# protocol/vdf

Hardware: AMD Instinct MI355X
Metric: MSM GPoints/s at 2^20 (Pallas, Pedersen-commitment MSM of Nova prove_step); prove_step/s in `prove_step` (higher is better)
Workload: dtype u32

## Files before the change

### bindings/rust/vdf-hip-sys/src/lib.rs

```rust
#![allow(non_camel_case_types, non_snake_case)]
use std::os::raw::{c_char, c_int, c_uint, c_void};

#[repr(C)] pub struct VdfCtx { _private: [u8; 0] }
#[repr(C)] pub struct VdfBases { _private: [u8; 0] }
#[repr(C)] pub struct VdfShape { _private: [u8; 0] }
#[repr(C)] pub struct VdfMsmJob { _private: [u8; 0] }
#[repr(C)] pub struct VdfPp { _private: [u8; 0] }
#[repr(C)] pub struct VdfCircuits { _private: [u8; 0] }
#[repr(C)] pub struct VdfProof { _private: [u8; 0] }
#[repr(C)] pub struct VdfSnark { _private: [u8; 0] }
#[repr(C)] pub struct VdfCs { _private: [u8; 0] }
#[repr(C)] pub struct VdfCustomChain { _private: [u8; 0] }

#[repr(C)] #[derive(Clone, Copy, Debug, PartialEq, Eq)] pub struct VdfFe { pub l: [u64; 4] }
#[repr(C)] #[derive(Clone, Copy, Debug, PartialEq, Eq)] pub struct VdfAffine { pub x: VdfFe, pub y: VdfFe }
#[repr(C)] #[derive(Clone, Copy, Debug, PartialEq, Eq)] pub struct VdfJac { pub x: VdfFe, pub y: VdfFe, pub z: VdfFe }
#[repr(C)] #[derive(Clone, Copy, Debug, PartialEq, Eq)] pub struct VdfState { pub x: VdfFe, pub y: VdfFe, pub i: VdfFe }
pub type VdfAllgatherFn = Option<unsafe extern "C" fn(user: *mut c_void, send: *const c_void, recv: *mut c_void, bytes: usize, stream: *mut c_void) -> c_int>;
#[repr(C)] #[derive(Clone, Copy)] pub struct VdfStepCircuit { pub arity: usize, pub synthesize: Option<unsafe extern "C" fn(self_: *mut c_void, cs: *mut VdfCs, z_in: *const u32, z_out: *mut u32) -> c_int>, pub self_: *mut c_void }
#[repr(C)] #[derive(Clone, Copy, Debug)] pub struct VdfNovaStepInfo { pub comm_W1: VdfAffine, pub X1: [VdfFe; 2], pub comm_T1: VdfAffine, pub comm_T2: VdfAffine, pub r1: [u64; 4], pub r2: [u64; 4] }
#[repr(C)] #[derive(Clone, Copy, Debug)] pub struct VdfNovaAugInputs { pub params: VdfFe, pub i: VdfFe, pub z0: [VdfFe; 3], pub zi: [VdfFe; 3], pub U_comm_W: VdfAffine, pub U_comm_E: VdfAffine, pub U_u: VdfFe, pub U_X: [VdfFe; 2], pub u_comm_W: VdfAffine, pub u_X: [VdfFe; 2], pub T: VdfAffine }
#[repr(C)] #[derive(Clone, Copy, Debug)] pub struct VdfKernelEvent { pub name: [c_char; 24], pub bytes: f64, pub start_ms: f64, pub end_ms: f64 }
#[repr(C)] #[derive(Clone, Copy, Debug)] pub struct VdfHipTuning { pub struct_size: u32, pub msm_direct: i32, pub direct_priority: i32, pub direct_fused: i32, pub light_priority: i32, pub accumulate_fill: i32, pub accumulate_lds: i32, pub slice_len: i32, pub part_bits: i32, pub reduction: i32, pub reduction_quads: i32, pub heavy_min: i32, pub giant_span: i32, pub nifs_lanes: i32, pub shim_cache: i32, pub nifs_fused: i32, pub fold_u128: i32, pub fixup_serial: i32, pub sort_staged: i32, pub glv: i32 }
#[repr(C)] #[derive(Clone, Copy, Debug)] pub struct VdfNovaTuning { pub struct_size: u32, pub flags: u32, pub digit_budget_bytes: u64, pub digit_window: i32, pub early_rows: i32, pub stencil: i32, pub small_window: i32, pub big_window: i32, pub packed_commit: i32, pub lookahead_early: i32, pub gate_accumulate: i32, pub fold_on_rows: i32, pub nifs_ahead: i32, pub early_row_parts: i32, pub lookahead_priority: i32, pub side_accumulate_fill: i32, pub verbose: i32, pub compress_queues: i32, pub rows_at_challenge: i32, pub fold_fused: i32, pub periodic_rows: i32, pub custom_ahead: i32 }
#[repr(C)] #[derive(Clone, Copy, Debug, PartialEq, Eq)] pub struct VdfNovaRoParams { pub struct_size: u32, pub family: i32, pub width: i32, pub full_rounds: i32, pub partial_rounds: i32, pub alpha: i32, pub challenge_bits: i32, pub hash_bits: i32 }
#[repr(C)] #[derive(Clone, Copy, Debug)] pub struct VdfIpaOpening { pub weight: VdfFe, pub k: c_int, pub log_m: c_int, pub lo: *const VdfFe, pub hi: *const VdfFe, pub pattern: *const VdfFe }
#[repr(C)] #[derive(Clone, Copy, Debug)] pub struct VdfNovaStreamStats { pub eval_ms: f64, pub after_eval_ms: f64, pub max_backlog: u64, pub steps: u64 }
#[repr(C)] #[derive(Clone, Copy, Debug, PartialEq, Eq)] pub struct VdfTapeOp { pub op: u8, pub dst: u8, pub a: u8, pub b: u8 }
#[repr(C)] #[derive(Clone, Copy, Debug)] pub struct VdfRoundTape { pub ops: *const VdfTapeOp, pub n_ops: usize, pub consts: *const VdfFe, pub n_consts: usize, pub n_slots: u32, pub n_vars: u32, pub n_cons: u32, pub n_inv: u32, pub n_adv: u32 }
#[repr(C)] #[derive(Clone, Copy)] pub struct VdfRoundBody { pub n_inv: usize, pub n_carry: usize, pub n_adv: usize, pub body: Option<unsafe extern "C" fn(self_: *mut c_void, cs: *mut VdfCs, j: u32, inv: *const u32, carry: *const u32, cur: *const u32, next: *const u32, carry_out: *mut u32) -> c_int>, pub self_: *mut c_void }
#[repr(C)] #[derive(Clone, Copy)] pub struct VdfWalkBody { pub n_inv: usize, pub n_adv: usize, pub body: Option<unsafe extern "C" fn(self_: *mut c_void, cs: *mut VdfCs, j: u32, inv: *const u32, next: *const u32, cur_out: *mut u32) -> c_int>, pub self_: *mut c_void }
#[repr(C)] #[derive(Clone, Copy, Debug, PartialEq, Eq)] pub struct VdfPeriodicTerm { pub kind: u8, pub c0: u8, pub c1: u8, pub pad: u8, pub col: u32 }
#[repr(C)] #[derive(Clone, Copy, Debug)] pub struct VdfPeriodicRows { pub n_cons: u32, pub n_vars: u32, pub j0: u64, pub row_start: *const u16, pub terms: *const VdfPeriodicTerm, pub n_terms: usize, pub consts: *const VdfFe, pub n_consts: usize }
#[repr(C)] #[derive(Clone, Copy, Debug, PartialEq, Eq)] pub struct VdfPowStep { pub src: u8, pub squarings: u8, pub mul: u8, pub dst: u8 }

#[link(name = "vdf_hip")]
extern "C" {
    pub fn vdf_ctx_create(device_ids: *const c_int, n_devices: c_int, out: *mut *mut VdfCtx) -> c_int;
// ... 287 lines not shown
```

### include/vdf_hip.h

```cpp
#ifndef VDF_HIP_H
#define VDF_HIP_H

#include <stdbool.h>
#include <stddef.h>
#include <stdint.h>

#ifdef __cplusplus
extern "C" {
#endif

typedef struct { uint64_t l[4]; } vdf_fe;
typedef struct { vdf_fe x, y; } vdf_affine;
typedef struct { vdf_fe x, y, z; } vdf_jac;
typedef struct { vdf_fe x, y, i; } vdf_state;

typedef struct vdf_ctx vdf_ctx;
typedef struct vdf_bases vdf_bases;
typedef struct vdf_shape vdf_shape;

enum {
  VDF_OK = 0,
  VDF_ERR_BAD_ARG = 1,
  VDF_ERR_BAD_LENGTH = 2,
  VDF_ERR_NONCANONICAL = 3,
// ... 246 lines not shown
  int32_t accumulate_fill;
  int32_t accumulate_lds;
  int32_t slice_len;
  int32_t part_bits;
  int32_t reduction;
  int32_t reduction_quads;
  int32_t heavy_min;
  int32_t giant_span;
  int32_t nifs_lanes;
  int32_t shim_cache;
  int32_t nifs_fused;
  int32_t fold_u128;
  int32_t fixup_serial;
  int32_t sort_staged;
  int32_t glv;
} vdf_hip_tuning;
int  vdf_hip_tuning_get(vdf_hip_tuning* out);
int  vdf_hip_tuning_set(const vdf_hip_tuning* in);
int  vdf_ctx_set_accumulate_fill(vdf_ctx* ctx, int workgroups_per_cu);
int  vdf_ctx_clock_probe(vdf_ctx* ctx, int iters, double* shader_mhz, double* kernel_ms);
int  vdf_dev_alloc(vdf_ctx* ctx, size_t bytes, void** out);
int  vdf_dev_free(vdf_ctx* ctx, void* p);
int  vdf_dev_mem_info(vdf_ctx* ctx, size_t* free_bytes, size_t* total_bytes);
int  vdf_dev_memcpy(vdf_ctx* ctx, void* dst, const void* src, size_t bytes);
int  vdf_ptr_download(void* dst, const void* src, size_t bytes);
int  vdf_host_alloc(vdf_ctx* ctx, size_t bytes, void** out);
int  vdf_host_free(vdf_ctx* ctx, void* p);
int  vdf_dev_memset(vdf_ctx* ctx, void* dst, int value, size_t bytes);
const char* vdf_version(void);

// ... 5 lines not shown
```

### vdf_amd/csrc/abi.hip

```cpp
#include <algorithm>
#include <cstring>
#include <cstdio>
#include <cstdlib>
#include <thread>
#include <functional>
#include <map>
#include <array>
#include <new>
#include <memory>
#include <atomic>
#include <deque>
#include <mutex>
#include <initializer_list>
#include <utility>
#include "internal.h"
#include "fe.cuh"

using vdf::Status;

namespace {

thread_local std::string g_create_err;
std::mutex g_default_mu;
vdf_ctx* g_default_ctx = nullptr;
// ... 76 lines not shown
  if (ctx) ctx->err = s.msg; else g_create_err = s.msg;
  return s.code;
}


std::once_flag g_tune_once;
std::mutex g_tune_mu;
std::deque<vdf_hip_tuning> g_tune_snapshots;
std::atomic<const vdf_hip_tuning*> g_tune{nullptr};
vdf_hip_tuning tuning_defaults() {
  vdf_hip_tuning t{};
  t.struct_size = (uint32_t)sizeof(vdf_hip_tuning);
  t.msm_direct = 1; t.direct_priority = 2; t.direct_fused = 1; t.light_priority = 3; t.accumulate_fill = 0;
  t.accumulate_lds = 0; t.slice_len = 0; t.part_bits = -1; t.reduction = 1; t.reduction_quads = 0; t.heavy_min = 0;
  t.giant_span = 0; t.nifs_lanes = 0; t.shim_cache = 0; t.nifs_fused = 1; t.fold_u128 = 1;
  t.fixup_serial = 1; t.sort_staged = 1; t.glv = 1;
  return t;
}
bool tuning_valid(const vdf_hip_tuning& t) {
  auto in = [](int v, int lo, int hi) { return v >= lo && v <= hi; };
  return in(t.msm_direct, 0, 1) && in(t.direct_priority, 0, 3) && in(t.direct_fused, 0, 1) && in(t.light_priority, 0, 3) &&
         in(t.accumulate_fill, 0, 3) && in(t.accumulate_lds, 0, 65536) && in(t.slice_len, 0, 65536) && in(t.part_bits, -1, 19) &&
         in(t.reduction, 0, 1) && (t.reduction_quads == 0 || in(t.reduction_quads, 64, 65536)) &&
         (t.heavy_min == 0 || in(t.heavy_min, 1, 4096)) && (t.giant_span == 0 || in(t.giant_span, 16, 1 << 20)) &&
         (t.nifs_lanes == 0 || t.nifs_lanes == 1 || t.nifs_lanes == 4 || t.nifs_lanes == 8) && in(t.shim_cache, 0, 64) &&
         in(t.nifs_fused, 0, 1) && in(t.fold_u128, 0, 1) && in(t.fixup_serial, 0, 1) && in(t.sort_staged, 0, 1) && in(t.glv, 0, 1);
}
void tuning_publish(const vdf_hip_tuning& t) {
  g_tune_snapshots.push_back(t);
  g_tune_snapshots.back().struct_size = (uint32_t)sizeof(vdf_hip_tuning);
  g_tune.store(&g_tune_snapshots.back(), std::memory_order_release);
}
void tuning_from_env() {
  vdf_hip_tuning t = tuning_defaults();
  const struct { const char* name; int32_t* field; } vars[] = {
      {"VDF_MSM_DIRECT", &t.msm_direct}, {"VDF_MSM_DIRECT_PRIO", &t.direct_priority}, {"VDF_MSM_DIRECT_FUSED", &t.direct_fused},
      {"VDF_MSM_LIGHT_PRIO", &t.light_priority}, {"VDF_MSM_ACC_WG", &t.accumulate_fill}, {"VDF_MSM_ACC_LDS", &t.accumulate_lds},
      {"VDF_MSM_L", &t.slice_len}, {"VDF_MSM_PB", &t.part_bits}, {"VDF_MSM_RED", &t.reduction},
      {"VDF_MSM_RED_QUADS", &t.reduction_quads}, {"VDF_MSM_HEAVY_MIN", &t.heavy_min}, {"VDF_MSM_GIANT_SPAN", &t.giant_span},
      {"VDF_NIFS_LANES", &t.nifs_lanes}, {"VDF_SHIM_CACHE", &t.shim_cache}, {"VDF_NIFS_FUSED", &t.nifs_fused}, {"VDF_FOLD_U128", &t.fold_u128},
      {"VDF_MSM_FIXUP_SERIAL", &t.fixup_serial}, {"VDF_MSM_SORT_STAGED", &t.sort_staged}, {"VDF_MSM_GLV", &t.glv}};
  for (const auto& v : vars) {
    const char* e = std::getenv(v.name);
    if (!e || !*e) continue;
    const int32_t old = *v.field;
    *v.field = (int32_t)std::atol(e);
    if (!tuning_valid(t)) *v.field = old;
  }
  std::lock_guard<std::mutex> lock(g_tune_mu);
  tuning_publish(t);
}
}
namespace vdf {
thread_local KSink* tl_ksink = nullptr;
const vdf_hip_tuning& tuning() {
  std::call_once(g_tune_once, tuning_from_env);
// ... 2211 lines not shown
```

### vdf_amd/csrc/msm.hip

```cpp
#include <cstdlib>
#include <cstring>
#include "internal.h"
#include "ec.cuh"
#include "ecq.cuh"

namespace vdf {

static constexpr uint32_t SIGN_BIT = 0x80000000u;

__device__ __forceinline__ void raise_wave_priority(int wave_prio = 3) {
  if (wave_prio >= 3) __builtin_amdgcn_s_setprio(3);
  else if (wave_prio == 2) __builtin_amdgcn_s_setprio(2);
  else if (wave_prio == 1) __builtin_amdgcn_s_setprio(1);
}
static constexpr int ACC_WG_PER_CU = 3;
static constexpr int ACC_WG_FILL = 2;
static constexpr uint32_t HEAVY_MIN = 6;
static constexpr uint32_t GIANT_SPAN = 64;
static constexpr uint32_t GIANT_CHUNK = 32;
static constexpr uint32_t GIANT_PARTS = 256;
static constexpr uint32_t MAX_GIANTS = 192;
__device__ __forceinline__ uint32_t giant_parts(uint32_t span) {
  const uint32_t p = (span + GIANT_CHUNK - 1) / GIANT_CHUNK;
  return p > GIANT_PARTS ? GIANT_PARTS : p;
// ... 228 lines not shown
      const uint32_t mag = d & ~SIGN_BIT;
      if (!mag) continue;
      const uint32_t s = (uint32_t)w % (uint32_t)sets, j = (uint32_t)w / (uint32_t)sets;
      const uint32_t bin = ((set0 + s) << pb) | ((mag - 1) >> fb);
      const uint32_t pos = atomicAdd(&cur[bin], 1u);
      if (SCATTER) { recsP[pos] = (j * tstride + pbase + i) | (d & SIGN_BIT); recsK[pos] = (uint16_t)((mag - 1) & fmask); }
    }
  }
  if (!SCATTER) {
    __syncthreads();
    for (uint32_t b = threadIdx.x; b < bins; b += 256) mine[b] = cur[b];
  }
}

static constexpr uint32_t PART_STAGE_BINS = 512;
template <class SP>
__global__ __launch_bounds__(256) void k_part_staged(PartGroups pg, int is_mont, int c, int windows, int sets, int pb, int fb,
                                                     uint32_t bins, uint32_t chA, uint32_t tstride,
                                                     const uint32_t* __restrict__ countsA, const uint32_t* __restrict__ pstart,
                                                     uint32_t* __restrict__ recsP, uint16_t* __restrict__ recsK, int wave_prio) {
  raise_wave_priority(wave_prio);
  __shared__ uint32_t limbs[9 * 256];
  __shared__ uint32_t cur[PART_STAGE_BINS];
  __shared__ uint32_t tcnt[PART_STAGE_BINS];
  __shared__ uint32_t toff[PART_STAGE_BINS + 1];
  __shared__ uint32_t tpos[PART_STAGE_BINS];
  __shared__ uint32_t stage[256 * 16];
  __shared__ uint32_t skb[256 * 16];
  const uint32_t* mine = countsA + (size_t)blockIdx.x * bins;
  for (uint32_t b = threadIdx.x; b < bins; b += 256) { cur[b] = pstart[b] + mine[b]; tcnt[b] = 0; }
  int g = 0;
// ... 3 lines not shown
  const uint32_t n = pg.n[g];
  const uint32_t lo = (blockIdx.x - blk0) * chA;
  const uint32_t hi = (lo + chA < n) ? lo + chA : n;
  const uint32_t fmask = (1u << fb) - 1u;
  const uint32_t set0 = (uint32_t)g * (uint32_t)sets;
  const uint32_t pbase = pg.off[g];
  const uint32_t per_lane = (bins + 63) / 64;
  Fe<SP> nxt = fe_zero<SP>();
  if (lo + threadIdx.x < hi) nxt = fe_load<SP>(scalars + (size_t)(lo + threadIdx.x) * 8);
  __syncthreads();
  for (uint32_t base = lo; base < hi; base += 256) {
    const uint32_t i = base + threadIdx.x;
    Fe<SP> mags = nxt;
    if (i + 256 < hi) nxt = fe_load<SP>(scalars + (size_t)(i + 256) * 8);
    uint32_t ssign = 0;
    if (i < hi) {
      if (pg.signed_scalars) { ssign = mags.v[7] & SIGN_BIT; mags.v[7] &= ~SIGN_BIT; }
      stage_scalar<SP>(limbs, mags, is_mont);
      DigitIter it{limbs + threadIdx.x, 0u};
      for (int w = 0; w < windows; ++w) {
        const uint32_t mag = it.next(w, c) & ~SIGN_BIT;
        if (!mag) continue;
        atomicAdd(&tcnt[((set0 + (uint32_t)w % (uint32_t)sets) << pb) | ((mag - 1) >> fb)], 1u);
      }
    }
    __syncthreads();
    if (threadIdx.x < 64) {
      uint32_t run = 0;
      const uint32_t b0 = threadIdx.x * per_lane;
      for (uint32_t k = 0; k < per_lane; ++k) if (b0 + k < bins) run += tcnt[b0 + k];
      uint32_t incl = run;
#pragma unroll
      for (int d = 1; d < 64; d <<= 1) { const uint32_t o = __shfl_up(incl, d, 64); if ((int)threadIdx.x >= d) incl += o; }
      uint32_t off = incl - run;
      for (uint32_t k = 0; k < per_lane; ++k) if (b0 + k < bins) { toff[b0 + k] = off; tpos[b0 + k] = off; off += tcnt[b0 + k]; }
      if (threadIdx.x == 63) toff[bins] = incl;
    }
    __syncthreads();
    if (i < hi) {
      DigitIter it{limbs + threadIdx.x, 0u};
      for (int w = 0; w < windows; ++w) {
        const uint32_t d = it.next(w, c) ^ ssign;
        const uint32_t mag = d & ~SIGN_BIT;
        if (!mag) continue;
        const uint32_t s = (uint32_t)w % (uint32_t)sets, j = (uint32_t)w / (uint32_t)sets;
        const uint32_t bin = ((set0 + s) << pb) | ((mag - 1) >> fb);
        const uint32_t p = atomicAdd(&tpos[bin], 1u);
        stage[p] = (j * tstride + pbase + i) | (d & SIGN_BIT);
        skb[p] = ((mag - 1) & fmask) | (bin << 16);
      }
    }
    __syncthreads();
    const uint32_t tile_n = toff[bins];
    for (uint32_t q = threadIdx.x; q < tile_n; q += 256) {
// ... 364 lines not shown
      if (!queued) q.items[atomicAdd(q.count, 1u)] = g;
    }
    return;
  }
  QPoint<P> acc = qpoint_load_lazy<P>(bucket_acc + (size_t)g * 128);
  QPoint<P> nxt = qpoint_load_lazy<P>(heads + (size_t)(tf + 1) * 128);
  for (uint32_t t = tf + 1; t <= tl; ++t) {
    const QPoint<P> cur = nxt;
    if (t < tl) nxt = qpoint_load_lazy<P>(heads + (size_t)(t + 1) * 128);
    acc = qpoint_add<P>(acc, cur);
  }
  qpoint_store<P>(bucket_acc + (size_t)g * 128, acc);
}

template <class P>
__global__ __launch_bounds__(256) void k_fixup_serial(const uint32_t* __restrict__ bstart, uint32_t nkeys, uint32_t slots,
                                                      uint32_t Lfixed, char* __restrict__ bucket_acc,
                                                      const char* __restrict__ heads, uint32_t* __restrict__ heavy,
                                                      uint32_t heavy_min, uint32_t giant_span, int wave_prio) {
  raise_wave_priority(wave_prio);
  const uint32_t g = blockIdx.x * 256 + threadIdx.x;
  if (g >= nkeys) return;
  const uint32_t ne = bstart[nkeys];
  const uint32_t L = slice_len(ne, slots, Lfixed);
  const uint32_t s = bstart[g], e = bstart[g + 1];
  if (e <= s) return;
  const uint32_t tf = s / L, tl = (e - 1) / L;
  if (tl == tf) return;
  uint32_t heavy_span = 2u * ((ne / nkeys + L - 1) / L) + 4u;
  if (heavy_span < heavy_min) heavy_span = heavy_min;
  if (tl - tf > heavy_span) {
    const HeavyLayout q = heavy_layout(heavy, nkeys);
    bool queued = false;
    if (tl - tf > giant_span) {
      const uint32_t idx = atomicAdd(q.giant_count, 1u);
      if (idx < MAX_GIANTS) { q.giants[idx] = g; queued = true; }
    }
    if (!queued) q.items[atomicAdd(q.count, 1u)] = g;
    return;
  }
  XYZZ<P> acc = xyzz_load<P>(bucket_acc + (size_t)g * 128);
  bool have = !fe_is_zero(acc.zz), flip = false;
  if (have) { acc.x = fe_canon(acc.x); acc.y = fe_canon(acc.y); acc.zz = fe_canon(acc.zz); acc.zzz = fe_canon(acc.zzz); }
  XYZZ<P> nxt = xyzz_load<P>(heads + (size_t)(tf + 1) * 128);
  for (uint32_t t = tf + 1; t <= tl; ++t) {
    XYZZ<P> cur = nxt;
    if (t < tl) nxt = xyzz_load<P>(heads + (size_t)(t + 1) * 128);
    if (fe_is_zero(cur.zz)) continue;
    cur.x = fe_canon(cur.x); cur.y = fe_canon(cur.y); cur.zz = fe_canon(cur.zz); cur.zzz = fe_canon(cur.zzz);
    if (have && flip) cur.y = fe_neg_nz(cur.y);
    xyzz_add_lazy<P>(acc, have, flip, cur);
  }
  xyzz_store<P>(bucket_acc + (size_t)g * 128, xyzz_lazy_resolve<P>(acc, have, flip));
}

template <class P>
__global__ __launch_bounds__(64) void k_fixup_heavy(const uint32_t* __restrict__ bstart, uint32_t nkeys, uint32_t slots,
                                                    uint32_t Lfixed, char* __restrict__ bucket_acc,
                                                    const char* __restrict__ heads, uint32_t* __restrict__ heavy,
                                                    char* __restrict__ giant, int wave_prio) {
  raise_wave_priority(wave_prio);
  const HeavyLayout q = heavy_layout(heavy, nkeys);
  const uint32_t count = *q.count;
  uint32_t ngiant = *q.giant_count;
  if (ngiant > MAX_GIANTS) ngiant = MAX_GIANTS;
  if (count == 0 && ngiant == 0) return;
  const uint32_t L = slice_len(bstart[nkeys], slots, Lfixed);
  const uint32_t quad = threadIdx.x >> 2;
// ... 120 lines not shown
    const uint32_t l = sidx - nrows;
    for (uint32_t h = qi; h < nrows; h += Q) acc = qpoint_add<P>(acc, qpoint_load_lazy<P>(bp + ((size_t)h * ncols + l) * 128));
  }
  qpoint_store<P>(lds_raw + (size_t)lt * 128, acc);
  __syncthreads();
  for (uint32_t stride = Q >> 1; stride >= 1; stride >>= 1) {
    if (qi < stride) {
      acc = qpoint_add<P>(acc, qpoint_load<P>(lds_raw + (size_t)(lt + stride) * 128));
      qpoint_store<P>(lds_raw + (size_t)lt * 128, acc);
    }
    __syncthreads();
  }
  if (qi == 0 && sidx < nsums) qpoint_store<P>(sums + ((size_t)set * nsums + sidx) * 128, acc);
}

template <class P>
__global__ __launch_bounds__(256) void k_red_weights(const char* __restrict__ sums, uint32_t nbk, uint32_t Lb, uint32_t bA,
                                                     uint32_t bB, char* __restrict__ partials, int wave_prio) {
  raise_wave_priority(wave_prio);
  __shared__ __align__(16) char lds_raw[64 * 128];
  const uint32_t ncols = 1u << Lb, nrows = nbk >> Lb, nsums = nrows + ncols;
  const uint32_t set = blockIdx.x / (bA + bB), blk = blockIdx.x % (bA + bB);
  const uint32_t lt = threadIdx.x >> 2;
  const bool col = blk < bA;
  const uint32_t idx = (col ? blk : blk - bA) * 64 + lt;
  const uint32_t weight = col ? idx + 1 : idx;
  QPoint<P> tot = qpoint_identity<P>();
  if (idx < (col ? ncols : nrows) && weight) {
    const QPoint<P> pt = qpoint_load<P>(sums + ((size_t)set * nsums + (col ? nrows + idx : idx)) * 128);
    const QPoint<P> mpt = qpoint_neg<P>(pt);
// ... 449 lines not shown
__global__ __launch_bounds__(256) void k_precompute(const char* __restrict__ pts, uint32_t n, int shift, int tables,
                                                    char* __restrict__ table) {
  const uint32_t i = blockIdx.x * 256 + threadIdx.x;
  if (i >= n) return;
  Affine<P> a = affine_load<P>(pts + (size_t)i * 64);
  affine_store<P>(table + (size_t)i * 64, a);
  XYZZ<P> r = xyzz_from_affine(a);
  for (int j = 1; j < tables; ++j) {
    for (int k = 0; k < shift; ++k) r = xyzz_dbl(r);
    Affine<P> o = xyzz_to_affine(r);
    affine_store<P>(table + ((size_t)j * n + i) * 64, o);
    r = xyzz_from_affine(o);
  }
}

template <class P>
static Status msm_tail_t(int c, int sets, int groups, uint32_t nbk, const char* bucket_acc, char* partials, char* wsum,
                         void* d_out, hipStream_t st, int prio) {
  const uint32_t gsets = (uint32_t)(groups * sets);
  if (use_matrix_reduction(nbk)) {
    const MatGeom g = mat_geom(gsets, nbk);
    char* sums = partials;
    char* parts = partials + g.sums_bytes;
    hipLaunchKernelGGL((k_red_sums<P>), dim3(gsets * g.wgs_per_set), dim3(256), 0, st, bucket_acc, nbk, g.Lb, g.Q, g.wgs_per_set, sums, prio);
    hipLaunchKernelGGL((k_red_weights<P>), dim3(gsets * (g.bA + g.bB)), dim3(256), 0, st, sums, nbk, g.Lb, g.bA, g.bB, parts, prio);
    char* direct = sets == 1 ? bytes_of(d_out) : nullptr;
    hipLaunchKernelGGL((k_red_combine<P>), dim3(gsets), dim3(256), 0, st, parts, g.Lb, g.bA, g.bB, wsum, direct, prio);
    if (direct) {
      VDF_TRY_HIP(hipGetLastError());
      return Status{};
    }
  } else {
    const RedGeom rg = red_geom((size_t)gsets * nbk, nbk);
    hipLaunchKernelGGL((k_reduce1<P>), dim3(gsets * rg.blocks_per_set), dim3(rg.block * 4), (size_t)rg.block * 128, st,
                       bucket_acc, nbk, rg.seg, rg.threads_per_set, rg.blocks_per_set, partials, prio);
    hipLaunchKernelGGL((k_reduce2<P>), dim3(gsets), dim3(256), 0, st, partials, rg.blocks_per_set, wsum, prio);
  }
  hipLaunchKernelGGL((k_final<P>), dim3(groups), dim3(64), 0, st, wsum, sets, c, bytes_of(d_out), prio);
  VDF_TRY_HIP(hipGetLastError());
// ... 23 lines not shown
  pg.groups = p.groups;
  pg.signed_scalars = p.signed_scalars ? 1 : 0;
  for (int g = 0; g < p.groups; ++g) {
    pg.scalars[g] = reinterpret_cast<const uint32_t*>(d_scalars[g]);
    pg.n[g] = p.gn[g]; pg.off[g] = p.goff[g]; pg.blk_end[g] = p.gblk_end[g];
  }
  const size_t lds_bins = (size_t)p.bins * 4;

  if (ev) VDF_TRY_HIP(hipEventRecord(ev[0], st));
  {
  KTimer kt(st, "msm_sort(5 launches)", 0.0);
  hipLaunchKernelGGL((k_part<SP, false>), dim3(p.nblkA), dim3(256), lds_bins, st, pg, is_mont ? 1 : 0, p.c, p.windows,
                     p.sets, p.pb, p.fb, p.bins, p.chA, p.tstride, countsA, pstart, recsP, recsK, prio);
  hipLaunchKernelGGL(k_part_scan, dim3(p.bins), dim3(256), 0, st, countsA, p.bins, p.nblkA, pcount, heavy, heavy + 1 + nkeys + 2, prio);
  hipLaunchKernelGGL(k_scan_keys, dim3(1), dim3(1024), 0, st, pcount, p.bins, pstart, prio);
  if (tuning().sort_staged && p.bins <= PART_STAGE_BINS && p.windows <= 16)
    hipLaunchKernelGGL((k_part_staged<SP>), dim3(p.nblkA), dim3(256), 0, st, pg, is_mont ? 1 : 0, p.c, p.windows,
                       p.sets, p.pb, p.fb, p.bins, p.chA, p.tstride, countsA, pstart, recsP, recsK, prio);
  else
    hipLaunchKernelGGL((k_part<SP, true>), dim3(p.nblkA), dim3(256), lds_bins, st, pg, is_mont ? 1 : 0, p.c, p.windows,
                       p.sets, p.pb, p.fb, p.bins, p.chA, p.tstride, countsA, pstart, recsP, recsK, prio);
  if (tuning().sort_staged && nf <= 256)
    hipLaunchKernelGGL(k_fine_staged<4>, dim3(p.bins), dim3(1024), 0, st, recsP, recsK, pstart, p.bins, nf, bstart, sorted, bucket_acc, p.slots, p.Lfixed,
                       reinterpret_cast<uint32_t*>(base + w.tstart), prio);
  else if (tuning().sort_staged)
    hipLaunchKernelGGL(k_fine_staged<8>, dim3(p.bins), dim3(1024), 0, st, recsP, recsK, pstart, p.bins, nf, bstart, sorted, bucket_acc, p.slots, p.Lfixed,
                       reinterpret_cast<uint32_t*>(base + w.tstart), prio);
  else
    hipLaunchKernelGGL(k_fine, dim3(p.bins), dim3(1024), 0, st, recsP, recsK, pstart, p.bins, nf, bstart, sorted, bucket_acc, p.slots, p.Lfixed,
                       reinterpret_cast<uint32_t*>(base + w.tstart), prio);
  }
  if (ev) VDF_TRY_HIP(hipEventRecord(ev[1], st));
  if (acc_gate) VDF_TRY_HIP(hipStreamWaitEvent(st, acc_gate, 0));
  {
  KTimer kt(st, "k_accumulate", 96.0 * p.n);
  const unsigned acc_lds = (unsigned)(tuning().accumulate_lds >= 0 && tuning().accumulate_lds <= 65536 ? tuning().accumulate_lds : 0);
  hipLaunchKernelGGL((k_accumulate<P>), dim3((p.nthreads + 255) / 256), dim3(256), acc_lds, st, sorted, bstart, nkeys,
                     reinterpret_cast<const uint32_t*>(base + w.tstart), cbytes_of(d_points), bucket_acc, heads, p.slots, p.Lfixed, p.nthreads);
  }
  if (ev) VDF_TRY_HIP(hipEventRecord(ev[2], st));
  const FixupTune tune = fixup_tune();
  KTimer kt_tail(st, ext_bucket_acc ? "msm_fixup(2 launches)" : "msm_tail(fixup+reduce)", 0.0);
  if (tuning().fixup_serial)
    hipLaunchKernelGGL((k_fixup_serial<P>), dim3((nkeys + 255) / 256), dim3(256), 0, st, bstart, nkeys, p.slots, p.Lfixed, bucket_acc, heads,
                       heavy, tune.heavy_min, tune.giant_span, prio);
  else
    hipLaunchKernelGGL((k_fixup<P>), dim3((nkeys * 4 + 255) / 256), dim3(256), 0, st, bstart, nkeys, p.slots, p.Lfixed, bucket_acc, heads,
                       heavy, tune.heavy_min, tune.giant_span, prio);
  hipLaunchKernelGGL((k_fixup_heavy<P>), dim3(16 * GIANT_PARTS), dim3(64), 0, st, bstart, nkeys, p.slots, p.Lfixed, bucket_acc, heads, heavy,
                     base + w.giant, prio);
  if (!ext_bucket_acc) VDF_TRY(msm_tail_t<P>(p.c, p.sets, p.groups, p.nbk, bucket_acc, partials, wsum, d_out, st, prio));
  if (ev) VDF_TRY_HIP(hipEventRecord(ev[3], st));
  VDF_TRY_HIP(hipGetLastError());
  return Status{};
}

Status msm_run(int curve, const MsmPlan& plan, const void* d_points, const void* const* d_scalars, bool is_mont, void* ws,
               void* d_out, hipStream_t stream, hipEvent_t* ev, void* ext_bucket_acc, hipEvent_t acc_gate, int prio) {
  char* ext = bytes_of(ext_bucket_acc);
  prio = std::min(prio, (int)tuning().light_priority);
  return with_curve(curve, [&](auto base, auto scalar) {
    return msm_run_t<tag_t<decltype(base)>, tag_t<decltype(scalar)>>(plan, d_points, d_scalars, is_mont, ws, d_out, stream, ev, ext, acc_gate, prio);
  });
}

static size_t tail_scratch_bytes(size_t gsets, uint32_t nbk) {
  const RedGeom rg = red_geom(gsets * nbk, nbk);
  const size_t seg = align_up(gsets * rg.blocks_per_set * 128, 256), mat = mat_geom(gsets, nbk).scratch_bytes;
  return seg > mat ? seg : mat;
}
size_t msm_tail_ws_bytes(int groups, int sets, uint32_t nbk) {
  const size_t gsets = (size_t)groups * sets;
  return align_up(gsets * nbk * 128, 256) + tail_scratch_bytes(gsets, nbk) + align_up(gsets * 128, 256);
}
Status msm_tail(int curve, int c, int sets, int groups, uint32_t nbk, void* tail_ws, void* d_out, hipStream_t stream, int prio) {
  const size_t gsets = (size_t)groups * sets;
  prio = std::min(prio, (int)tuning().light_priority);
  char* bucket_acc = bytes_of(tail_ws);
  char* partials = bucket_acc + align_up(gsets * nbk * 128, 256);
  char* wsum = partials + tail_scratch_bytes(gsets, nbk);
  return with_curve(curve, [&](auto base, auto) {
    return msm_tail_t<tag_t<decltype(base)>>(c, sets, groups, nbk, bucket_acc, partials, wsum, d_out, stream, prio);
  });
}

template <class P>
__global__ __launch_bounds__(64) void k_point_sum(const char* __restrict__ pts, uint32_t n, char* __restrict__ out, int wave_prio) {
  raise_wave_priority(wave_prio);
  const uint32_t quad = threadIdx.x >> 2;
  QPoint<P> acc = qpoint_identity<P>();
  for (uint32_t i = quad; i < n; i += 16) {
    Jac<P> j;
    j.x = fe_load<P>(pts + (size_t)i * 96);
    j.y = fe_load<P>(pts + (size_t)i * 96 + 32);
    j.z = fe_load<P>(pts + (size_t)i * 96 + 64);
    acc = qpoint_add<P>(acc, qpoint_scatter(jac_to_xyzz(j)));
  }
// ... 81 lines not shown
```

### vdf_amd/hip.py

```python
from __future__ import annotations

import ctypes as C
import weakref
from typing import Optional, Sequence, Tuple

import numpy as np

from . import _lib
from ._lib import lib, CURVE_PALLAS, CURVE_VESTA, FIELD_FP, FIELD_FQ


class HipTuning(C.Structure):
    _fields_ = [("struct_size", C.c_uint32)] + [(k, C.c_int32) for k in (
        "msm_direct", "direct_priority", "direct_fused", "light_priority", "accumulate_fill", "accumulate_lds", "slice_len", "part_bits",
        "reduction", "reduction_quads", "heavy_min", "giant_span", "nifs_lanes", "shim_cache", "nifs_fused", "fold_u128", "fixup_serial", "sort_staged", "glv")]


def tuning_get() -> HipTuning:
    t = HipTuning()
    rc = lib.vdf_hip_tuning_get(C.byref(t))
    if rc != 0:
        raise VdfError(rc, "vdf_hip_tuning_get")
    return t


def tuning_set(**fields) -> HipTuning:
    t = tuning_get()
    for k, v in fields.items():
        if k not in dict(HipTuning._fields_):
            raise KeyError(k)
# ... 644 lines not shown
```

Baseline: 1.082.

## Record partition digits in registers and add span-sorted fixup and run-based reduction

The staged partition kernel gets window-count template specialisations that keep each thread's bucket keys and payloads in registers from the counting pass, so the second pass no longer re-extracts scalar digits. These specialisations are used by default for large single-group MSMs. A tail_serial tuning flag, off by default, also enables a fixup kernel that sorts buckets by span within a workgroup to even out per-thread serial work, plus a reduction kernel that sums contiguous runs of buckets serially and then tree-reduces them in LDS. The register records cost extra VGPRs per window, which can lower occupancy.

```diff
diff --git a/bindings/rust/vdf-hip-sys/src/lib.rs b/bindings/rust/vdf-hip-sys/src/lib.rs
--- a/bindings/rust/vdf-hip-sys/src/lib.rs
+++ b/bindings/rust/vdf-hip-sys/src/lib.rs
@@ -21,7 +21,7 @@
 #[repr(C)] #[derive(Clone, Copy, Debug)] pub struct VdfNovaStepInfo { pub comm_W1: VdfAffine, pub X1: [VdfFe; 2], pub comm_T1: VdfAffine, pub comm_T2: VdfAffine, pub r1: [u64; 4], pub r2: [u64; 4] }
 #[repr(C)] #[derive(Clone, Copy, Debug)] pub struct VdfNovaAugInputs { pub params: VdfFe, pub i: VdfFe, pub z0: [VdfFe; 3], pub zi: [VdfFe; 3], pub U_comm_W: VdfAffine, pub U_comm_E: VdfAffine, pub U_u: VdfFe, pub U_X: [VdfFe; 2], pub u_comm_W: VdfAffine, pub u_X: [VdfFe; 2], pub T: VdfAffine }
 #[repr(C)] #[derive(Clone, Copy, Debug)] pub struct VdfKernelEvent { pub name: [c_char; 24], pub bytes: f64, pub start_ms: f64, pub end_ms: f64 }
-#[repr(C)] #[derive(Clone, Copy, Debug)] pub struct VdfHipTuning { pub struct_size: u32, pub msm_direct: i32, pub direct_priority: i32, pub direct_fused: i32, pub light_priority: i32, pub accumulate_fill: i32, pub accumulate_lds: i32, pub slice_len: i32, pub part_bits: i32, pub reduction: i32, pub reduction_quads: i32, pub heavy_min: i32, pub giant_span: i32, pub nifs_lanes: i32, pub shim_cache: i32, pub nifs_fused: i32, pub fold_u128: i32, pub fixup_serial: i32, pub sort_staged: i32, pub glv: i32 }
+#[repr(C)] #[derive(Clone, Copy, Debug)] pub struct VdfHipTuning { pub struct_size: u32, pub msm_direct: i32, pub direct_priority: i32, pub direct_fused: i32, pub light_priority: i32, pub accumulate_fill: i32, pub accumulate_lds: i32, pub slice_len: i32, pub part_bits: i32, pub reduction: i32, pub reduction_quads: i32, pub heavy_min: i32, pub giant_span: i32, pub nifs_lanes: i32, pub shim_cache: i32, pub nifs_fused: i32, pub fold_u128: i32, pub fixup_serial: i32, pub sort_staged: i32, pub glv: i32, pub tail_serial: i32 }
 #[repr(C)] #[derive(Clone, Copy, Debug)] pub struct VdfNovaTuning { pub struct_size: u32, pub flags: u32, pub digit_budget_bytes: u64, pub digit_window: i32, pub early_rows: i32, pub stencil: i32, pub small_window: i32, pub big_window: i32, pub packed_commit: i32, pub lookahead_early: i32, pub gate_accumulate: i32, pub fold_on_rows: i32, pub nifs_ahead: i32, pub early_row_parts: i32, pub lookahead_priority: i32, pub side_accumulate_fill: i32, pub verbose: i32, pub compress_queues: i32, pub rows_at_challenge: i32, pub fold_fused: i32, pub periodic_rows: i32, pub custom_ahead: i32 }
 #[repr(C)] #[derive(Clone, Copy, Debug, PartialEq, Eq)] pub struct VdfNovaRoParams { pub struct_size: u32, pub family: i32, pub width: i32, pub full_rounds: i32, pub partial_rounds: i32, pub alpha: i32, pub challenge_bits: i32, pub hash_bits: i32 }
 #[repr(C)] #[derive(Clone, Copy, Debug)] pub struct VdfIpaOpening { pub weight: VdfFe, pub k: c_int, pub log_m: c_int, pub lo: *const VdfFe, pub hi: *const VdfFe, pub pattern: *const VdfFe }
diff --git a/include/vdf_hip.h b/include/vdf_hip.h
--- a/include/vdf_hip.h
+++ b/include/vdf_hip.h
@@ -284,6 +284,7 @@
   int32_t fixup_serial;
   int32_t sort_staged;
   int32_t glv;
+  int32_t tail_serial;
 } vdf_hip_tuning;
 int  vdf_hip_tuning_get(vdf_hip_tuning* out);
 int  vdf_hip_tuning_set(const vdf_hip_tuning* in);
diff --git a/vdf_amd/csrc/abi.hip b/vdf_amd/csrc/abi.hip
--- a/vdf_amd/csrc/abi.hip
+++ b/vdf_amd/csrc/abi.hip
@@ -114,7 +114,7 @@
   t.msm_direct = 1; t.direct_priority = 2; t.direct_fused = 1; t.light_priority = 3; t.accumulate_fill = 0;
   t.accumulate_lds = 0; t.slice_len = 0; t.part_bits = -1; t.reduction = 1; t.reduction_quads = 0; t.heavy_min = 0;
   t.giant_span = 0; t.nifs_lanes = 0; t.shim_cache = 0; t.nifs_fused = 1; t.fold_u128 = 1;
-  t.fixup_serial = 1; t.sort_staged = 1; t.glv = 1;
+  t.fixup_serial = 1; t.sort_staged = 1; t.glv = 1; t.tail_serial = 0;
   return t;
 }
 bool tuning_valid(const vdf_hip_tuning& t) {
@@ -124,7 +124,8 @@
          in(t.reduction, 0, 1) && (t.reduction_quads == 0 || in(t.reduction_quads, 64, 65536)) &&
          (t.heavy_min == 0 || in(t.heavy_min, 1, 4096)) && (t.giant_span == 0 || in(t.giant_span, 16, 1 << 20)) &&
          (t.nifs_lanes == 0 || t.nifs_lanes == 1 || t.nifs_lanes == 4 || t.nifs_lanes == 8) && in(t.shim_cache, 0, 64) &&
-         in(t.nifs_fused, 0, 1) && in(t.fold_u128, 0, 1) && in(t.fixup_serial, 0, 1) && in(t.sort_staged, 0, 1) && in(t.glv, 0, 1);
+         in(t.nifs_fused, 0, 1) && in(t.fold_u128, 0, 1) && in(t.fixup_serial, 0, 1) && in(t.sort_staged, 0, 1) && in(t.glv, 0, 1) &&
+         in(t.tail_serial, 0, 1);
 }
 void tuning_publish(const vdf_hip_tuning& t) {
   g_tune_snapshots.push_back(t);
@@ -139,7 +140,8 @@
       {"VDF_MSM_L", &t.slice_len}, {"VDF_MSM_PB", &t.part_bits}, {"VDF_MSM_RED", &t.reduction},
       {"VDF_MSM_RED_QUADS", &t.reduction_quads}, {"VDF_MSM_HEAVY_MIN", &t.heavy_min}, {"VDF_MSM_GIANT_SPAN", &t.giant_span},
       {"VDF_NIFS_LANES", &t.nifs_lanes}, {"VDF_SHIM_CACHE", &t.shim_cache}, {"VDF_NIFS_FUSED", &t.nifs_fused}, {"VDF_FOLD_U128", &t.fold_u128},
-      {"VDF_MSM_FIXUP_SERIAL", &t.fixup_serial}, {"VDF_MSM_SORT_STAGED", &t.sort_staged}, {"VDF_MSM_GLV", &t.glv}};
+      {"VDF_MSM_FIXUP_SERIAL", &t.fixup_serial}, {"VDF_MSM_SORT_STAGED", &t.sort_staged}, {"VDF_MSM_GLV", &t.glv},
+      {"VDF_MSM_TAIL_SERIAL", &t.tail_serial}};
   for (const auto& v : vars) {
     const char* e = std::getenv(v.name);
     if (!e || !*e) continue;
diff --git a/vdf_amd/csrc/msm.hip b/vdf_amd/csrc/msm.hip
--- a/vdf_amd/csrc/msm.hip
+++ b/vdf_amd/csrc/msm.hip
@@ -266,7 +266,8 @@
 }
 
 static constexpr uint32_t PART_STAGE_BINS = 512;
-template <class SP>
+static constexpr uint32_t PART_NO_RECORD = 0xFFFFFFFFu;
+template <class SP, int WINDOWS>
 __global__ __launch_bounds__(256) void k_part_staged(PartGroups pg, int is_mont, int c, int windows, int sets, int pb, int fb,
                                                      uint32_t bins, uint32_t chA, uint32_t tstride,
                                                      const uint32_t* __restrict__ countsA, const uint32_t* __restrict__ pstart,
@@ -300,14 +301,34 @@
     Fe<SP> mags = nxt;
     if (i + 256 < hi) nxt = fe_load<SP>(scalars + (size_t)(i + 256) * 8);
     uint32_t ssign = 0;
+    constexpr int NREC = WINDOWS > 0 ? WINDOWS : 1;
+    uint32_t rkb[NREC], rpay[NREC];
+    if constexpr (WINDOWS > 0) {
+#pragma unroll
+      for (int w = 0; w < WINDOWS; ++w) rkb[w] = PART_NO_RECORD;
+    }
     if (i < hi) {
       if (pg.signed_scalars) { ssign = mags.v[7] & SIGN_BIT; mags.v[7] &= ~SIGN_BIT; }
       stage_scalar<SP>(limbs, mags, is_mont);
       DigitIter it{limbs + threadIdx.x, 0u};
-      for (int w = 0; w < windows; ++w) {
-        const uint32_t mag = it.next(w, c) & ~SIGN_BIT;
-        if (!mag) continue;
-        atomicAdd(&tcnt[((set0 + (uint32_t)w % (uint32_t)sets) << pb) | ((mag - 1) >> fb)], 1u);
+      if constexpr (WINDOWS > 0) {
+#pragma unroll
+        for (int w = 0; w < WINDOWS; ++w) {
+          const uint32_t d = it.next(w, c) ^ ssign;
+          const uint32_t mag = d & ~SIGN_BIT;
+          if (!mag) continue;
+          const uint32_t s = (uint32_t)w % (uint32_t)sets, j = (uint32_t)w / (uint32_t)sets;
+          const uint32_t bin = ((set0 + s) << pb) | ((mag - 1) >> fb);
+          rkb[w] = ((mag - 1) & fmask) | (bin << 16);
+          rpay[w] = (j * tstride + pbase + i) | (d & SIGN_BIT);
+          atomicAdd(&tcnt[bin], 1u);
+        }
+      } else {
+        for (int w = 0; w < windows; ++w) {
+          const uint32_t mag = it.next(w, c) & ~SIGN_BIT;
+          if (!mag) continue;
+          atomicAdd(&tcnt[((set0 + (uint32_t)w % (uint32_t)sets) << pb) | ((mag - 1) >> fb)], 1u);
+        }
       }
     }
     __syncthreads();
@@ -323,7 +344,15 @@
       if (threadIdx.x == 63) toff[bins] = incl;
     }
     __syncthreads();
-    if (i < hi) {
+    if constexpr (WINDOWS > 0) {
+#pragma unroll
+      for (int w = 0; w < WINDOWS; ++w) {
+        if (rkb[w] == PART_NO_RECORD) continue;
+        const uint32_t p = atomicAdd(&tpos[rkb[w] >> 16], 1u);
+        stage[p] = rpay[w];
+        skb[p] = rkb[w];
+      }
+    } else if (i < hi) {
       DigitIter it{limbs + threadIdx.x, 0u};
       for (int w = 0; w < windows; ++w) {
         const uint32_t d = it.next(w, c) ^ ssign;
@@ -718,6 +747,23 @@
 }
 
 template <class P>
+__device__ __forceinline__ void fixup_bucket_serial(char* __restrict__ bucket, const char* __restrict__ heads, uint32_t tf, uint32_t tl) {
+  XYZZ<P> acc = xyzz_load<P>(bucket);
+  bool have = !fe_is_zero(acc.zz), flip = false;
+  if (have) { acc.x = fe_canon(acc.x); acc.y = fe_canon(acc.y); acc.zz = fe_canon(acc.zz); acc.zzz = fe_canon(acc.zzz); }
+  XYZZ<P> nxt = xyzz_load<P>(heads + (size_t)(tf + 1) * 128);
+  for (uint32_t t = tf + 1; t <= tl; ++t) {
+    XYZZ<P> cur = nxt;
+    if (t < tl) nxt = xyzz_load<P>(heads + (size_t)(t + 1) * 128);
+    if (fe_is_zero(cur.zz)) continue;
+    cur.x = fe_canon(cur.x); cur.y = fe_canon(cur.y); cur.zz = fe_canon(cur.zz); cur.zzz = fe_canon(cur.zzz);
+    if (have && flip) cur.y = fe_neg_nz(cur.y);
+    xyzz_add_lazy<P>(acc, have, flip, cur);
+  }
+  xyzz_store<P>(bucket, xyzz_lazy_resolve<P>(acc, have, flip));
+}
+
+template <class P>
 __global__ __launch_bounds__(256) void k_fixup_serial(const uint32_t* __restrict__ bstart, uint32_t nkeys, uint32_t slots,
                                                       uint32_t Lfixed, char* __restrict__ bucket_acc,
                                                       const char* __restrict__ heads, uint32_t* __restrict__ heavy,
@@ -743,19 +789,73 @@
     if (!queued) q.items[atomicAdd(q.count, 1u)] = g;
     return;
   }
-  XYZZ<P> acc = xyzz_load<P>(bucket_acc + (size_t)g * 128);
-  bool have = !fe_is_zero(acc.zz), flip = false;
-  if (have) { acc.x = fe_canon(acc.x); acc.y = fe_canon(acc.y); acc.zz = fe_canon(acc.zz); acc.zzz = fe_canon(acc.zzz); }
-  XYZZ<P> nxt = xyzz_load<P>(heads + (size_t)(tf + 1) * 128);
-  for (uint32_t t = tf + 1; t <= tl; ++t) {
-    XYZZ<P> cur = nxt;
-    if (t < tl) nxt = xyzz_load<P>(heads + (size_t)(t + 1) * 128);
-    if (fe_is_zero(cur.zz)) continue;
-    cur.x = fe_canon(cur.x); cur.y = fe_canon(cur.y); cur.zz = fe_canon(cur.zz); cur.zzz = fe_canon(cur.zzz);
-    if (have && flip) cur.y = fe_neg_nz(cur.y);
-    xyzz_add_lazy<P>(acc, have, flip, cur);
-  }
-  xyzz_store<P>(bucket_acc + (size_t)g * 128, xyzz_lazy_resolve<P>(acc, have, flip));
+  fixup_bucket_serial<P>(bucket_acc + (size_t)g * 128, heads, tf, tl);
+}
+
+static constexpr uint32_t FIXUP_EVEN_PASSES = 1;
+static constexpr uint32_t FIXUP_EVEN_TILE = 256 * FIXUP_EVEN_PASSES;
+template <class P>
+__global__ __launch_bounds__(256) void k_fixup_even(const uint32_t* __restrict__ bstart, uint32_t nkeys, uint32_t slots,
+                                                    uint32_t Lfixed, char* __restrict__ bucket_acc,
+                                                    const char* __restrict__ heads, uint32_t* __restrict__ heavy,
+                                                    uint32_t heavy_min, uint32_t giant_span, int wave_prio) {
+  raise_wave_priority(wave_prio);
+  __shared__ uint32_t hist[64];
+  __shared__ uint32_t order[FIXUP_EVEN_TILE];
+  __shared__ uint32_t ospan[FIXUP_EVEN_TILE];
+  const uint32_t ne = bstart[nkeys];
+  const uint32_t L = slice_len(ne, slots, Lfixed);
+  uint32_t heavy_span = 2u * ((ne / nkeys + L - 1) / L) + 4u;
+  if (heavy_span < heavy_min) heavy_span = heavy_min;
+  if (threadIdx.x < 64) hist[threadIdx.x] = 0;
+  __syncthreads();
+  uint32_t adds[FIXUP_EVEN_PASSES], rank[FIXUP_EVEN_PASSES];
+#pragma unroll
+  for (uint32_t k = 0; k < FIXUP_EVEN_PASSES; ++k) {
+    const uint32_t g = blockIdx.x * FIXUP_EVEN_TILE + k * 256 + threadIdx.x;
+    adds[k] = 0;
+    if (g < nkeys) {
+      const uint32_t s = bstart[g], e = bstart[g + 1];
+      if (e > s) {
+        const uint32_t span = (e - 1) / L - s / L;
+        if (span > heavy_span) {
+          const HeavyLayout q = heavy_layout(heavy, nkeys);
+          bool queued = false;
+          if (span > giant_span) {
+            const uint32_t idx = atomicAdd(q.giant_count, 1u);
+            if (idx < MAX_GIANTS) { q.giants[idx] = g; queued = true; }
+          }
+          if (!queued) q.items[atomicAdd(q.count, 1u)] = g;
+        } else {
+          adds[k] = span;
+        }
+      }
+    }
+    rank[k] = atomicAdd(&hist[adds[k] < 63u ? adds[k] : 63u], 1u);
+  }
+  __syncthreads();
+  if (threadIdx.x < 64) {
+    const uint32_t cnt = hist[threadIdx.x];
+    uint32_t incl = cnt;
+#pragma unroll
+    for (int d = 1; d < 64; d <<= 1) { const uint32_t o = __shfl_up(incl, d, 64); if ((int)threadIdx.x >= d) incl += o; }
+    hist[threadIdx.x] = incl - cnt;
+  }
+  __syncthreads();
+#pragma unroll
+  for (uint32_t k = 0; k < FIXUP_EVEN_PASSES; ++k) {
+    const uint32_t at = hist[adds[k] < 63u ? adds[k] : 63u] + rank[k];
+    order[at] = k * 256 + threadIdx.x;
+    ospan[at] = adds[k];
+  }
+  __syncthreads();
+  for (uint32_t k = 0; k < FIXUP_EVEN_PASSES; ++k) {
+    const uint32_t span = ospan[k * 256 + threadIdx.x];
+    if (span == 0) continue;
+    const uint32_t g = blockIdx.x * FIXUP_EVEN_TILE + order[k * 256 + threadIdx.x];
+    const uint32_t tf = bstart[g] / L;
+    fixup_bucket_serial<P>(bucket_acc + (size_t)g * 128, heads, tf, tf + span);
+  }
 }
 
 template <class P>
@@ -906,6 +1006,67 @@
   if (qi == 0 && sidx < nsums) qpoint_store<P>(sums + ((size_t)set * nsums + sidx) * 128, acc);
 }
 
+#ifndef VDF_RED_RUN
+#define VDF_RED_RUN 4
+#endif
+static constexpr uint32_t RED_RUN = VDF_RED_RUN;
+static_assert(RED_RUN == 4 || RED_RUN == 8 || RED_RUN == 16, "the run length of k_red_sums_runs");
+struct RunGeom { uint32_t wgs_rows, wgs_cols; bool ok; };
+static RunGeom run_geom(const MatGeom& g) {
+  RunGeom r;
+  const uint32_t run_r = g.ncols < RED_RUN ? g.ncols : RED_RUN, run_c = g.nrows < RED_RUN ? g.nrows : RED_RUN;
+  r.wgs_rows = (g.nrows * (g.ncols / run_r) + 255) / 256;
+  r.wgs_cols = (g.ncols * (g.nrows / run_c) + 255) / 256;
+  r.ok = g.ncols / run_r <= 256 && g.nrows / run_c <= 256;
+  return r;
+}
+template <class P>
+__global__ __launch_bounds__(256) void k_red_sums_runs(const char* __restrict__ bucket_acc, uint32_t nbk, uint32_t Lb, uint32_t wgs_rows,
+                                                       uint32_t wgs_cols, char* __restrict__ sums, int wave_prio) {
+  raise_wave_priority(wave_prio);
+  __shared__ __align__(16) char lds_raw[256 * 128];
+  const uint32_t ncols = 1u << Lb, nrows = nbk >> Lb, nsums = nrows + ncols;
+  const uint32_t set = blockIdx.x / (wgs_rows + wgs_cols), blk = blockIdx.x % (wgs_rows + wgs_cols);
+  const bool col = blk >= wgs_rows;
+  const uint32_t len = col ? nrows : ncols, count = col ? ncols : nrows;
+  const uint32_t run = len < RED_RUN ? len : RED_RUN;
+  const uint32_t per = len / run;
+  const uint32_t pid0 = (col ? blk - wgs_rows : blk) * 256;
+  const uint32_t sidx = (pid0 + threadIdx.x) / per, j = (pid0 + threadIdx.x) % per;
+  XYZZ<P> acc = xyzz_identity<P>();
+  bool have = false, flip = false;
+  if (sidx < count) {
+    const size_t first = col ? (size_t)j * run * ncols + sidx : (size_t)sidx * ncols + (size_t)j * run;
+    const size_t stride = col ? (size_t)ncols * 128 : 128;
+    const char* bp = bucket_acc + ((size_t)set * nbk + first) * 128;
+    XYZZ<P> nxt = xyzz_load<P>(bp);
+    for (uint32_t k = 0; k < run; ++k) {
+      XYZZ<P> cur = nxt;
+      if (k + 1 < run) nxt = xyzz_load<P>(bp + (size_t)(k + 1) * stride);
+      if (fe_is_zero(cur.zz)) continue;
+      cur.x = fe_canon(cur.x); cur.y = fe_canon(cur.y); cur.zz = fe_canon(cur.zz); cur.zzz = fe_canon(cur.zzz);
+      if (have && flip) cur.y = fe_neg_nz(cur.y);
+      xyzz_add_lazy<P>(acc, have, flip, cur);
+    }
+  }
+  xyzz_store<P>(lds_raw + (size_t)threadIdx.x * 128, xyzz_lazy_resolve<P>(acc, have, flip));
+  __syncthreads();
+  const uint32_t lt = threadIdx.x >> 2;
+  for (uint32_t cnt = per; cnt > 1; cnt >>= 1) {
+    const uint32_t half = cnt >> 1, nadd = (256 / per) * half;
+    for (uint32_t a = lt; a < nadd; a += 64) {
+      char* slot = lds_raw + ((size_t)(a / half) * per + a % half) * 128;
+      const QPoint<P> x = qpoint_load_lazy<P>(slot), y = qpoint_load_lazy<P>(slot + (size_t)half * 128);
+      qpoint_store<P>(slot, qpoint_add<P>(x, y));
+    }
+    __syncthreads();
+  }
+  for (uint32_t s = lt; s < 256 / per; s += 64) {
+    const uint32_t out = pid0 / per + s;
+    if (out < count) qpoint_store<P>(sums + ((size_t)set * nsums + (col ? nrows + out : out)) * 128, qpoint_load_lazy<P>(lds_raw + (size_t)s * per * 128));
+  }
+}
+
 template <class P>
 __global__ __launch_bounds__(256) void k_red_weights(const char* __restrict__ sums, uint32_t nbk, uint32_t Lb, uint32_t bA,
                                                      uint32_t bB, char* __restrict__ partials, int wave_prio) {
@@ -1385,15 +1546,22 @@
   }
 }
 
+static bool tail_serial_forms() { return tuning().tail_serial == 1; }
+
 template <class P>
 static Status msm_tail_t(int c, int sets, int groups, uint32_t nbk, const char* bucket_acc, char* partials, char* wsum,
-                         void* d_out, hipStream_t st, int prio) {
+                         void* d_out, hipStream_t st, int prio, bool runs) {
   const uint32_t gsets = (uint32_t)(groups * sets);
   if (use_matrix_reduction(nbk)) {
     const MatGeom g = mat_geom(gsets, nbk);
     char* sums = partials;
     char* parts = partials + g.sums_bytes;
-    hipLaunchKernelGGL((k_red_sums<P>), dim3(gsets * g.wgs_per_set), dim3(256), 0, st, bucket_acc, nbk, g.Lb, g.Q, g.wgs_per_set, sums, prio);
+    const RunGeom rg = run_geom(g);
+    if (runs && rg.ok)
+      hipLaunchKernelGGL((k_red_sums_runs<P>), dim3(gsets * (rg.wgs_rows + rg.wgs_cols)), dim3(256), 0, st, bucket_acc, nbk, g.Lb, rg.wgs_rows,
+                         rg.wgs_cols, sums, prio);
+    else
+      hipLaunchKernelGGL((k_red_sums<P>), dim3(gsets * g.wgs_per_set), dim3(256), 0, st, bucket_acc, nbk, g.Lb, g.Q, g.wgs_per_set, sums, prio);
     hipLaunchKernelGGL((k_red_weights<P>), dim3(gsets * (g.bA + g.bB)), dim3(256), 0, st, sums, nbk, g.Lb, g.bA, g.bB, parts, prio);
     char* direct = sets == 1 ? bytes_of(d_out) : nullptr;
     hipLaunchKernelGGL((k_red_combine<P>), dim3(gsets), dim3(256), 0, st, parts, g.Lb, g.bA, g.bB, wsum, direct, prio);
@@ -1447,10 +1615,19 @@
                      p.sets, p.pb, p.fb, p.bins, p.chA, p.tstride, countsA, pstart, recsP, recsK, prio);
   hipLaunchKernelGGL(k_part_scan, dim3(p.bins), dim3(256), 0, st, countsA, p.bins, p.nblkA, pcount, heavy, heavy + 1 + nkeys + 2, prio);
   hipLaunchKernelGGL(k_scan_keys, dim3(1), dim3(1024), 0, st, pcount, p.bins, pstart, prio);
-  if (tuning().sort_staged && p.bins <= PART_STAGE_BINS && p.windows <= 16)
-    hipLaunchKernelGGL((k_part_staged<SP>), dim3(p.nblkA), dim3(256), 0, st, pg, is_mont ? 1 : 0, p.c, p.windows,
-                       p.sets, p.pb, p.fb, p.bins, p.chA, p.tstride, countsA, pstart, recsP, recsK, prio);
-  else
+  if (tuning().sort_staged && p.bins <= PART_STAGE_BINS && p.windows <= 16) {
+#define VDF_PART_STAGED(W)                                                                                                       \
+  case W:                                                                                                                        \
+    hipLaunchKernelGGL((k_part_staged<SP, W>), dim3(p.nblkA), dim3(256), 0, st, pg, is_mont ? 1 : 0, p.c, p.windows, p.sets, p.pb, \
+                       p.fb, p.bins, p.chA, p.tstride, countsA, pstart, recsP, recsK, prio);                                     \
+    break;
+    const bool built_in = p.groups == 1 && (size_t)p.n * p.windows >= ((size_t)1 << 22);
+    switch (built_in ? p.windows : 0) {
+      VDF_PART_STAGED(13) VDF_PART_STAGED(14) VDF_PART_STAGED(15) VDF_PART_STAGED(16)
+      default: VDF_PART_STAGED(0)
+    }
+#undef VDF_PART_STAGED
+  } else
     hipLaunchKernelGGL((k_part<SP, true>), dim3(p.nblkA), dim3(256), lds_bins, st, pg, is_mont ? 1 : 0, p.c, p.windows,
                        p.sets, p.pb, p.fb, p.bins, p.chA, p.tstride, countsA, pstart, recsP, recsK, prio);
   if (tuning().sort_staged && nf <= 256)
@@ -1474,7 +1651,21 @@
   if (ev) VDF_TRY_HIP(hipEventRecord(ev[2], st));
   const FixupTune tune = fixup_tune();
   KTimer kt_tail(st, ext_bucket_acc ? "msm_fixup(2 launches)" : "msm_tail(fixup+reduce)", 0.0);
-  if (tuning().fixup_serial)
+  const bool serial_forms = tail_serial_forms();
+#ifdef VDF_TAIL_NO_EVEN
+  const bool even_form = false;
+#else
+  const bool even_form = serial_forms;
+#endif
+#ifdef VDF_TAIL_NO_RUNS
+  const bool runs_form = false;
+#else
+  const bool runs_form = serial_forms;
+#endif
+  if (tuning().fixup_serial && even_form)
+    hipLaunchKernelGGL((k_fixup_even<P>), dim3((nkeys + FIXUP_EVEN_TILE - 1) / FIXUP_EVEN_TILE), dim3(256), 0, st, bstart, nkeys, p.slots, p.Lfixed,
+                       bucket_acc, heads, heavy, tune.heavy_min, tune.giant_span, prio);
+  else if (tuning().fixup_serial)
     hipLaunchKernelGGL((k_fixup_serial<P>), dim3((nkeys + 255) / 256), dim3(256), 0, st, bstart, nkeys, p.slots, p.Lfixed, bucket_acc, heads,
                        heavy, tune.heavy_min, tune.giant_span, prio);
   else
@@ -1482,7 +1673,7 @@
                        heavy, tune.heavy_min, tune.giant_span, prio);
   hipLaunchKernelGGL((k_fixup_heavy<P>), dim3(16 * GIANT_PARTS), dim3(64), 0, st, bstart, nkeys, p.slots, p.Lfixed, bucket_acc, heads, heavy,
                      base + w.giant, prio);
-  if (!ext_bucket_acc) VDF_TRY(msm_tail_t<P>(p.c, p.sets, p.groups, p.nbk, bucket_acc, partials, wsum, d_out, st, prio));
+  if (!ext_bucket_acc) VDF_TRY(msm_tail_t<P>(p.c, p.sets, p.groups, p.nbk, bucket_acc, partials, wsum, d_out, st, prio, runs_form));
   if (ev) VDF_TRY_HIP(hipEventRecord(ev[3], st));
   VDF_TRY_HIP(hipGetLastError());
   return Status{};
@@ -1513,7 +1704,7 @@
   char* partials = bucket_acc + align_up(gsets * nbk * 128, 256);
   char* wsum = partials + tail_scratch_bytes(gsets, nbk);
   return with_curve(curve, [&](auto base, auto) {
-    return msm_tail_t<tag_t<decltype(base)>>(c, sets, groups, nbk, bucket_acc, partials, wsum, d_out, stream, prio);
+    return msm_tail_t<tag_t<decltype(base)>>(c, sets, groups, nbk, bucket_acc, partials, wsum, d_out, stream, prio, tail_serial_forms());
   });
 }
 
diff --git a/vdf_amd/hip.py b/vdf_amd/hip.py
--- a/vdf_amd/hip.py
+++ b/vdf_amd/hip.py
@@ -13,7 +13,8 @@
 class HipTuning(C.Structure):
     _fields_ = [("struct_size", C.c_uint32)] + [(k, C.c_int32) for k in (
         "msm_direct", "direct_priority", "direct_fused", "light_priority", "accumulate_fill", "accumulate_lds", "slice_len", "part_bits",
-        "reduction", "reduction_quads", "heavy_min", "giant_span", "nifs_lanes", "shim_cache", "nifs_fused", "fold_u128", "fixup_serial", "sort_staged", "glv")]
+        "reduction", "reduction_quads", "heavy_min", "giant_span", "nifs_lanes", "shim_cache", "nifs_fused", "fold_u128", "fixup_serial", "sort_staged", "glv",
+        "tail_serial")]
 
 
 def tuning_get() -> HipTuning:
```

New measurement: 1.090, median of 6. About the same (+0.7%).
